# peterdavidfagan/mujoco_robot_environments

Measured on AMD Instinct MI355X. Metric: env steps/sec (whole node), RearrangementEnv batch=4096 at 1/2/4/8 MI355X, higher is better.
Workload: dtype f32

## Files before the change

include/mre.h:

```cpp
#ifndef MRE_H
#define MRE_H
#include <stddef.h>
#include <stdint.h>
#ifdef __cplusplus
extern "C" {
#endif

#define MRE_NQ 43
#define MRE_NV 39
#define MRE_NU 8
#define MRE_NQ_PAD 44
#define MRE_TRACE_W 88
#define MRE_TRACE_QVEL 48
#define MRE_NV_PAD 40
#define MRE_MAX_PROPS 4

typedef enum {
  MRE_OK = 0,
  MRE_ERR_ARG = -1,
  MRE_ERR_MODEL = -2,
  MRE_ERR_HIP = -3,
  MRE_ERR_NOGPU = -4
} mre_status;

// ... 107 lines not shown

#define MRE_SRC_RED 0
#define MRE_SRC_GREEN 1
#define MRE_SRC_BLUE 2
#define MRE_SRC_HEIGHT 3
#define MRE_F32 0
#define MRE_BF16 1
int mre_warp_inputs(void* stream, const float* hmap, const uint8_t* cmap, int n, int in_h, int in_w,
                    const int32_t* index, const float* mats, int samples, int out_h, int out_w,
                    int channels, const int32_t* chan_src, const float* chan_scale, const float* chan_bias,
                    int dtype, void* out);

int mre_correlate_workspace(int n, int rotations, int h, int w, size_t* bytes);
int mre_correlate(void* stream, const uint16_t* scene, const uint16_t* kern, int n, int rotations, int depth,
                  int h, int w, int crop, int dtype, void* logits, int64_t* best_index, float* best_value,
                  void* workspace, size_t workspace_bytes);

#define MRE_SOLVER_PGS 0
#define MRE_SOLVER_NEWTON 2
int mre_set_solver(mre_env*, int solver);
int mre_get_solver(mre_env*);
int mre_get_fallback_stats(mre_env*, long long* out4);
int mre_get_queue_info(mre_env*, long long* out5);

int mre_profile_enable(mre_env*, int on);
int mre_profile_read(mre_env*, float* total_ms, int* launches);

#ifdef __cplusplus
}
#endif
#endif
```

mujoco_robot_environments_amd/csrc/mre_api.cpp:

```cpp
#include <hip/hip_runtime.h>

#include <cmath>
#include <cstdio>
#include <cstdlib>
#include <cstring>
#include <string>
#include <algorithm>
#include <vector>

#include "mre_env.h"
#include "mre_labels.h"
#include "mre_heightmap.h"
#include "mre_warp.h"
#include "mre_warp_inputs.h"
#include "mre_correlate.h"
#include "mre_launch.h"
#include "mre_model.h"
#include "mre_records.h"

using namespace mre;

static thread_local std::string g_err;
int mre::fail(int code, const std::string& msg) {
  g_err = msg;
// ... 722 lines not shown
  if (!e) return fail(MRE_ERR_ARG, "null handle");
  DRAIN(e);
  if (solver != MRE_SOLVER_PGS && solver != MRE_SOLVER_NEWTON)
    return fail(MRE_ERR_ARG, "mre_set_solver: solver is 0 (PGS) or 2 (Newton)");
  HIPCHK(hipSetDevice(e->device));
  HIPCHK(hipStreamSynchronize(e->stream));
  e->solver = solver;
  return MRE_OK;
}

extern "C" int mre_get_solver(mre_env* e) {
  if (!e) return fail(MRE_ERR_ARG, "null handle");
  return e->solver;
}

extern "C" int mre_get_queue_info(mre_env* e, long long* out5) {
  if (!e || !out5) return fail(MRE_ERR_ARG, "mre_get_queue_info: null");
  DRAIN(e);
  out5[0] = e->n_queue_launches; out5[1] = e->queue_waves; out5[2] = e->queue_ticks; out5[3] = e->queue_ok ? 1 : 0;
  out5[4] = e->n_handovers;
  return MRE_OK;
}

extern "C" int mre_get_fallback_stats(mre_env* e, long long* out4) {
  if (!e || !out4) return fail(MRE_ERR_ARG, "mre_get_fallback_stats: null");
  DRAIN(e);
  out4[0] = e->n_large; out4[1] = e->n_reruns; out4[2] = e->n_promotions; out4[3] = e->n_demotions;
  return MRE_OK;
}

extern "C" int mre_set_state(mre_env* e, const float* qpos, const float* qvel) {
  if (!e) return fail(MRE_ERR_ARG, "null handle");
  DRAIN(e);
  int rc = MRE_OK;
  if (qpos) rc = copy_in(e, e->qpos, qpos, (size_t)e->N * NQP * 4);
  if (!rc && qvel) rc = copy_in(e, e->qvel, qvel, (size_t)e->N * NVP * 4);
  if (!rc && qpos) {
    HIPCHK(hipMemset2DAsync(e->qfine, QFINE_ROW * 4, 0, QFINE * 2, (size_t)e->N, e->stream));
    HIPCHK(hipMemset2DAsync(e->qfine + QFINE_CUBE_Q, QFINE_ROW * 4, 0, (QFINE_CUBE_V - QFINE_CUBE_Q) * 4, (size_t)e->N, e->stream));
  }
  if (!rc && qvel) {
    HIPCHK(hipMemset2DAsync(e->qfine + QFINE / 2, QFINE_ROW * 4, 0, QFINE * 2, (size_t)e->N, e->stream));
    HIPCHK(hipMemset2DAsync(e->qfine + QFINE_CUBE_V, QFINE_ROW * 4, 0, (QFINE_ROW - QFINE_CUBE_V) * 4, (size_t)e->N, e->stream));
  }
  return rc;
}
// ... 691 lines not shown
```

mujoco_robot_environments_amd/csrc/mre_dev.h:

```cpp
#pragma once
#include <stdint.h>

namespace mre {

constexpr int NB = 20;
constexpr int NRB = 16;
constexpr int GRIP_BODY0 = 8;
constexpr int NV = 39;
constexpr int NRV = 15;
constexpr int NQ = 43;
constexpr int NQP = 44;
constexpr int TRACE_W = 88;
constexpr int TRACE_QVEL = 48;
constexpr int NVP = 40;
constexpr int NU = 8;
constexpr int QFINE = 32;
constexpr int QFINE_ROW = 96;
constexpr int QFINE_CUBE_Q = 32;
constexpr int QFINE_CUBE_V = 60;
static_assert(QFINE_CUBE_Q + 7 * 4 == QFINE_CUBE_V && QFINE_CUBE_V + 6 * 4 <= QFINE_ROW, "qfine row layout");
constexpr int NPROP = 4;
constexpr int NG = 20;
constexpr int PROP_GEOM0 = 12;
constexpr int NPAIR = 128;
// ... 186 lines not shown
  float* contacts_full;
  int* settle_steps;
  int min_settle_steps;
  const uint8_t* large;
  int want_large;
  float *sv_qpos, *sv_qvel, *sv_qacc_ws, *sv_qfine, *sv_ctrl;
  int* sv_nstep;
  uint32_t* sv_status;
  uint8_t* sv_converged;
  int* launch_info;
  uint8_t* pending;
  int* q_head;
  int* q_tail;
  int* q_buf;
  int* q_acc;
  int* q_done;
  int* q_started;
  const int* q_gen;
  int q_gen_expect;
  int q_wait;
  int* q_err;
  int q_nticks, q_shards, q_cap, q_stride;
  int q_lshards, q_capl;
};
constexpr int QUEUE_TICKS_MAX = 256;
constexpr int QUEUE_SHARDS_MAX = 32;
constexpr int QUEUE_LSHARDS_MAX = 16;

struct SearchArgs {
  const DevModel* M;
  int N;
  float* qpos;
  const int* nprops;
  const float* prop_size;
  const uint8_t* env_mask;
  const long long* env_ids;
  long long env_id_offset;
  unsigned long long seed;
  const int* prop;
  int fixed_prop;
  const double* bounds;
  double shared_bounds[6];
  const int* tick_base;
  long long tick0;
  int max_attempts;
  int yaw_mode;
// ... 60 lines not shown
```

mujoco_robot_environments_amd/csrc/mre_env.h:

```cpp
#pragma once
#include <hip/hip_runtime.h>

#include <string>
#include <utility>
#include <vector>

#include "../../include/mre.h"
#include "mre_dev.h"
#include "mre_policy.h"

#define HIPCHK(x)                                                                       \
  do {                                                                                  \
    hipError_t e_ = (x);                                                                \
    if (e_ != hipSuccess)                                                               \
      return mre::fail(MRE_ERR_HIP, std::string(#x) + ": " + hipGetErrorString(e_));    \
  } while (0)

struct mre_env {
  int N = 0, device = 0;
  hipStream_t stream = nullptr;
  mre::DevModel* dM = nullptr;
  mre::DevModel hM;
  int solver = MRE_SOLVER_PGS;
  float *qpos = nullptr, *qvel = nullptr, *qacc_ws = nullptr, *ctrl = nullptr;
// ... 76 lines not shown
  bool queue_ok = true;
  int queue_ticks = 200;
  int queue_waves = 0;
  int queue_shards = 16;
  int queue_lshards = 8;
  bool queue_test_serial = false;
  int queue_spare_large = 8;
  int queue_run_ticks = 100;
  int queue_min_ticks = 32;
  float tick_tail = 0.f;
  bool tick_tail_valid = false;
  float queue_tail_min = 1.45f;
  unsigned tail_samples = 0;
  std::vector<int> tail_scratch;
  int queue_large_waves_max = 0;
  int* h_qlist = nullptr;
  int* q_ws = nullptr;
  int* q_gen = nullptr;
  int* h_q_err = nullptr;
  int* h_qgrp_order = nullptr;
  long n_queue_launches = 0;
  long long n_handovers = 0;
  int queue_last_handovers = 0;
  static constexpr int RING = mre::policy::RING;
  int ring = 2;
  static constexpr int NSTAGE = mre::policy::NSTAGE;
  hipEvent_t ev_main = nullptr;
  float* seq_copy[RING + 1] = {nullptr, nullptr, nullptr, nullptr, nullptr};
  size_t seq_cap = 0;
  unsigned seq_calls = 0;
  double dbg_wait_s = 0, dbg_call_s = 0; long dbg_calls = 0;
  int calls_since_drain = 0, sync_streak = 0;
  bool broken = false;
};

namespace mre {
int fail(int code, const std::string& msg);
int sched_create(mre_env* e);
void sched_destroy(mre_env* e);
int launch_step(mre_env* e, const StepArgs& a, bool settle = false, bool pipeline_ok = true, bool allow_queue = false);
int drain(mre_env* e, bool api_call = false);
}
#define DRAIN(e) do { int rc_ = mre::drain(e, true); if (rc_) return rc_; } while (0)
#define DRAIN_PENDING(e) do { int rc_ = mre::drain(e, false); if (rc_) return rc_; } while (0)

inline int profile_events(mre_env* e, hipEvent_t* e0, hipEvent_t* e1) {
// ... 12 lines not shown
```

mujoco_robot_environments_amd/csrc/mre_kernels.hip:

```cpp
#include <hip/hip_runtime.h>

#include "mre_dev.h"
#include "mre_math.h"
#include "mre_collide.h"

namespace mre {
using ModelP = MRE_MODEL_PTR(DevModel);
#if defined(MRE_PHASE_STAMPS) && MRE_PHASE_STAMPS >= 4
__shared__ unsigned long long dbg_acc[4];
#endif

struct OscSm {
  float J[6][7], M[7][7], MiJt[7][6], Li[6][6], Lam[6][6], V[6][6], Jbar[7][6];
  float ep[3], eo[3], F[6], LF[6], tn[7], Jbt[6], xd[6], w[6];
};

struct alignas(8) Blk {
  uint16_t row0;
  uint8_t type, nrows;
  uint8_t rslot;
  uint8_t pa, pb;
  uint8_t primary : 4;
  uint8_t bslot : 4;
};
// ... 1248 lines not shown
    }
  }
  for (int k = 0; k < S; ++k) {
    const int sh = home + k < S ? home + k : home + k - S;
    const int r = queue_pop_shard(a, l, sh, env, tick);
    if (r != 0) { shard = sh; return r > 0; }
  }
  return false;
}
MRE_DEV void queue_push(const StepArgs& a, int l, int env, int tick, int shard) {
  __builtin_amdgcn_fence(__ATOMIC_RELEASE, "agent");
  asm volatile("s_waitcnt vmcnt(0)" ::: "memory");
  if (l == 0) {
    const int i = __hip_atomic_fetch_add(a.q_tail + shard * QUEUE_TICKS_MAX + tick, 1, __ATOMIC_RELAXED, __HIP_MEMORY_SCOPE_AGENT);
    __hip_atomic_store(q_bucket(a, tick, shard) + i, env + 1, __ATOMIC_RELAXED, __HIP_MEMORY_SCOPE_AGENT);
  }
}

template <bool QUEUE>
MRE_DEV void step_body(const StepArgs& a, Sm& s) {
  OscSm& osc = s.osc;
  const int l = threadIdx.x;
  int env = 0, qtick = 0, qshard = 0;
  if (!QUEUE) {
    if ((int)blockIdx.x >= a.N) return;
    env = a.env_order != nullptr ? a.env_order[blockIdx.x] : (int)blockIdx.x;
  }
  if (QUEUE && !Q_LARGE && l == 0) __hip_atomic_fetch_add(a.q_started, 1, __ATOMIC_RELAXED, __HIP_MEMORY_SCOPE_AGENT);
  if (QUEUE && Q_LARGE && a.q_wait != 0) {
    for (unsigned idle = 0; q_load(a.q_gen) != a.q_gen_expect; ++idle) {
      if (idle > 1024u) return;
      __builtin_amdgcn_s_sleep(127);
    }
  }
 for (;;) {
  if (QUEUE) {
    if (!queue_pop(a, l, (int)(blockIdx.x % (unsigned)(Q_LARGE ? a.q_lshards : a.q_shards)), env, qtick, qshard)) return;
    if (qtick > 0 || Q_LARGE) __builtin_amdgcn_fence(__ATOMIC_ACQUIRE, "agent");
  }
  const int step_lo = QUEUE ? qtick * a.control_steps : 0, step_hi = QUEUE ? step_lo + a.control_steps : a.nsteps;
  if (QUEUE && !Q_LARGE && qtick == 0 && a.large != nullptr && a.large[env] != 0) continue;
  if (!QUEUE || (!Q_LARGE && qtick == 0)) {
#define MRE_PASS_SKIP { if (QUEUE) { if (l == 0) __hip_atomic_fetch_add(a.q_done, 1, __ATOMIC_RELAXED, __HIP_MEMORY_SCOPE_AGENT); continue; } return; }
  if (!QUEUE && a.large != nullptr && (a.large[env] != 0) != (a.want_large != 0)) return;
  if (a.env_mask != nullptr && a.env_mask[env] == 0) {
    if (a.launch_info != nullptr && l < 4) a.launch_info[(size_t)env * 4 + l] = -1;
    MRE_PASS_SKIP;
  }
  if (a.pending != nullptr && a.pending[env] != 0) {
    if (a.launch_info != nullptr && l < 4) a.launch_info[(size_t)env * 4 + l] = l == 0 ? -2 : -1;
    MRE_PASS_SKIP;
  }
#undef MRE_PASS_SKIP
  }
  ModelP M = (ModelP)a.M;

  const bool save = a.sv_qpos != nullptr && step_lo == 0;
  if (l < NQP) {
    const float v = a.qpos[(size_t)env * NQP + l];
    s.qpos[l] = v;
    if (save) a.sv_qpos[(size_t)env * NQP + l] = v;
  }
  if (l < NVP) {
    const float v = a.qvel[(size_t)env * NVP + l], w = a.qacc_ws[(size_t)env * NVP + l];
    s.qvel[l] = v;
    s.qacc[l] = w;
    s.qfrc_con[l] = 0.f;
    if (save) { a.sv_qvel[(size_t)env * NVP + l] = v; a.sv_qacc_ws[(size_t)env * NVP + l] = w; }
  }
  if (l < QFINE) {
    const float v = a.qfine != nullptr ? a.qfine[(size_t)env * QFINE_ROW + l] : 0.f;
    s.qlo[l] = v;
    if (save && a.qfine != nullptr) a.sv_qfine[(size_t)env * QFINE_ROW + l] = v;
  }
  if (save && a.qfine != nullptr && l < QFINE_ROW - QFINE)
    a.sv_qfine[(size_t)env * QFINE_ROW + QFINE + l] = a.qfine[(size_t)env * QFINE_ROW + QFINE + l];
  float cube_lo_keep = 0.f;
  if (QUEUE && !Q_LARGE && a.qfine != nullptr && l < QFINE_ROW - QFINE) cube_lo_keep = a.qfine[(size_t)env * QFINE_ROW + QFINE + l];
  if (l < NU) {
    const float v = a.ctrl[(size_t)env * NU + l];
    s.ctrl[l] = v;
    if (save) a.sv_ctrl[(size_t)env * NU + l] = v;
  }
  if (save && l == 0) {
    if (a.nstep != nullptr) a.sv_nstep[env] = a.nstep[env];
    a.sv_status[env] = a.status[env];
    a.sv_converged[env] = a.converged != nullptr ? a.converged[env] : (uint8_t)0;
  }
  if (l == 0) { s.nprops = a.nprops[env]; s.overflow = 0; s.ncon = 0; s.nefc = 0; s.solver_iters = 0; }
#ifdef MRE_NEWTON
  if (l < 24) s.zrow[l] = 0.f;
#endif
  if (l < NPROP * 3) {
    const float sz = a.prop_size[(size_t)env * NPROP * 3 + l];
    s.prop_size[l / 3][l % 3] = sz;
  }
  MRE_SYNC();
  if (l < NPROP) {
    const float m = M->body_mass[NRB + l];
    const float* z = s.prop_size[l];
    s.prop_mass[l] = m;
    s.prop_inertia[l][0] = m / 3.f * (z[1] * z[1] + z[2] * z[2]);
    s.prop_inertia[l][1] = m / 3.f * (z[0] * z[0] + z[2] * z[2]);
    s.prop_inertia[l][2] = m / 3.f * (z[0] * z[0] + z[1] * z[1]);
  }
  MRE_SYNC();

#if defined(MRE_PHASE_STAMPS) && MRE_PHASE_STAMPS >= 4
  if (l < 4) dbg_acc[l] = 0ull;
#endif
#ifdef MRE_PHASE_STAMPS
  unsigned long long stamp_acc[4] = {0, 0, 0, 0};
  unsigned long long stamp_t = __builtin_amdgcn_s_memtime();
#endif
  bool arm_converged = ((a.flags & F_CONV_CONTINUE) != 0 || (QUEUE && qtick > 0)) && a.converged != nullptr && a.converged[env] != 0;
  float grip_cmd = 0.f;
  const OscConfig* oscp = a.osc + (size_t)env * a.osc_stride;
  int hw_ncon = 0, hw_nefc = 0, hw_nrrow = 0, hw_npp = 0;
  const unsigned long long launch_t0 = __builtin_amdgcn_s_memtime();
  if (a.mode == CTRL_OSC) {
    if (l < 16) s.osc_tgt[l] = a.osc_target[(size_t)env * 16 + l];
    grip_cmd = a.grip_closed[env] ? M->act_ctrlrange[NU - 1][1] : M->act_ctrlrange[NU - 1][0];
    MRE_SYNC();
  }
  int steps_done = 0;
  bool settled = false;
  for (int step = step_lo; step < step_hi; ++step) {
    MRE_STAMP(7);
    position_stage(M, s, l);
    MRE_STAMP(12);
    MRE_STAMP(13);
    gripper_local(M, s, l);
    if ((a.flags & F_NO_CONSTRAINTS) == 0) connect_rows_local(M, s, l);
    MRE_STAMP(14);
    crb_mass_matrix(M, s, l);
    MRE_SYNC();
#ifndef MRE_NEWTON
    factor_robot_regs(s.qM, s.qLD, s.qLDinv);
#endif
    MRE_STAMP(15);
    MRE_STAMP(0);

// ... 161 lines not shown
  }
  if (a.sites != nullptr && q_last) {
    float* o = a.sites + (size_t)env * 16;
    if (l < 3) o[l] = s.site_xpos[M->opt_rec.tcp_site][l];
    if (l >= 3 && l < 6) o[l] = s.site_xpos[M->opt_rec.eef_site][l - 3];
    if (l == 6) {
      float q[4];
      mat2q(q, s.site_xmat[0]);
      o[6] = q[0]; o[7] = q[1]; o[8] = q[2]; o[9] = q[3];
    }
  }
  if (hand_over) {
    if (a.qfine != nullptr && l < QFINE_ROW - QFINE) a.qfine[(size_t)env * QFINE_ROW + QFINE + l] = cube_lo_keep;
  } else {
    if (l < NQP) a.qpos[(size_t)env * NQP + l] = s.qpos[l];
    if (l < NVP) {
      a.qvel[(size_t)env * NVP + l] = s.qvel[l];
      a.qacc_ws[(size_t)env * NVP + l] = l < NV ? s.qacc[l] : 0.f;
    }
    if (l < QFINE && a.qfine != nullptr) a.qfine[(size_t)env * QFINE_ROW + l] = s.qlo[l];
    if (l < NU) a.ctrl[(size_t)env * NU + l] = s.ctrl[l];
  }
  const bool q_more = QUEUE && !hand_over && qtick + 1 < a.q_nticks;
  if (l == 0 && a.launch_info != nullptr) {
    int* li = a.launch_info + (size_t)env * 4;
    unsigned long long dt = (__builtin_amdgcn_s_memtime() - launch_t0) >> 10;
    int moved = 0;
    if (QUEUE) {
      int* qa = a.q_acc + (size_t)env * 4;
      if (qtick > 0 || Q_LARGE) {
        hw_ncon = max(hw_ncon, q_load(qa + 0) & 0xFFFF); hw_nefc = max(hw_nefc, q_load(qa + 1));
        hw_nrrow = max(hw_nrrow, q_load(qa + 2) & 0xFFFF); hw_npp = max(hw_npp, q_load(qa + 2) >> 16);
        dt += (unsigned long long)q_load(qa + 3);
        moved = q_load(qa + 0) >> 16;
      }
      if (hand_over) moved = 1;
      if (q_more || hand_over) { qa[0] = hw_ncon | (moved << 16); qa[1] = hw_nefc; qa[2] = hw_nrrow | (hw_npp << 16); qa[3] = (int)dt; }
      else dt /= (unsigned long long)(qtick + 1);
    }
    if (!q_more && !hand_over) {
#ifdef MRE_LARGE_CAPS
      li[0] = (s.overflow ? 2 : 0) | (moved ? 4 : 0);
#else
      li[0] = s.overflow ? 1 : 0;
#endif
      li[1] = hw_ncon | ((int)(dt < 0x7FFFull ? dt : 0x7FFFull) << 16); li[2] = hw_nefc; li[3] = hw_nrrow | (hw_npp << 16);
    }
  }
#ifndef MRE_LARGE_CAPS
  if (!QUEUE && l == 0 && a.pending != nullptr && s.overflow) a.pending[env] = 1;
#endif
  if (l == 0 && a.status != nullptr && !hand_over) {
    unsigned st = 0;
    for (int k = 0; k < NQ; k++) if (!isfinite(s.qpos[k])) st |= 2u;
    if (s.overflow) st |= 4u;
    if (QUEUE) { if (st) __hip_atomic_fetch_or(a.status + env, st, __ATOMIC_RELAXED, __HIP_MEMORY_SCOPE_AGENT); }
    else a.status[env] |= st;
    if (a.stats != nullptr && a.nsteps > 0) {
      a.stats[env * 4 + 0] = s.ncon; a.stats[env * 4 + 1] = s.nefc;
      a.stats[env * 4 + 2] = s.solver_iters; a.stats[env * 4 + 3] = s.nl;
#ifdef MRE_PHASE_STAMPS
      for (int k = 0; k < 4; k++) a.stats[env * 4 + k] = (int)(stamp_acc[k] >> 4);
#if MRE_PHASE_STAMPS >= 4
      for (int k = 0; k < 4; k++) a.stats[env * 4 + k] = (int)(dbg_acc[k] >> 4);
#endif
#endif
    }
  }
  if (!QUEUE) return;
  if (hand_over) queue_push(a, l, env, qtick, a.q_shards + env % a.q_lshards);
  else if (q_more) queue_push(a, l, env, qtick + 1, qshard);
  else if (l == 0) __hip_atomic_fetch_add(a.q_done, 1, __ATOMIC_RELAXED, __HIP_MEMORY_SCOPE_AGENT);
 }
}

#ifdef MRE_NEWTON
#define MRE_VARIANT(name) name##_newton
#else
#define MRE_VARIANT(name) name
#endif

#ifdef MRE_LARGE_CAPS
__global__ __launch_bounds__(64, 2) void MRE_VARIANT(k_step_large)(StepArgs a) {
  __shared__ Sm s;
  step_body<false>(a, s);
}
}

extern "C" void MRE_VARIANT(mre_launch_step_large)(const mre::StepArgs* args, hipStream_t stream) {
  hipLaunchKernelGGL(mre::MRE_VARIANT(k_step_large), dim3(args->N), dim3(64), 0, stream, *args);
}
namespace mre {
// ... 379 lines not shown
```

mujoco_robot_environments_amd/csrc/mre_policy.h:

```cpp
#pragma once
#include <algorithm>

#include "mre_dev.h"

namespace mre {
namespace policy {

constexpr int RING = 4;
constexpr int NSTAGE = RING + 1;

inline int info_duration(const int* li) { return li[0] < 0 ? 0 : (li[1] >> 16); }

inline int compact_nrrow_max(bool newton) { return newton ? NRROW_MAX_COMPACT_NEWTON : NRROW_MAX_COMPACT_PGS; }
inline bool near_compact_caps(bool newton, int hw_ncon, int hw_nefc, int hw_nrrow, int hw_npp) {
  return 8 * hw_ncon > 7 * NCON_MAX || 8 * hw_nefc > 7 * NEFC_MAX || 8 * hw_nrrow > 7 * compact_nrrow_max(newton) || 8 * hw_npp > 7 * NPP_MAX;
}
inline bool far_below_compact_caps(bool newton, int hw_ncon, int hw_nefc, int hw_nrrow, int hw_npp) {
  return 8 * hw_ncon <= 5 * NCON_MAX && 8 * hw_nefc <= 5 * NEFC_MAX && 8 * hw_nrrow <= 5 * compact_nrrow_max(newton) && 8 * hw_npp <= 5 * NPP_MAX;
}

enum Action {
  NONE,
  RERUN,
  PROMOTE,
// ... 45 lines not shown
  return fs;
}

inline int queue_large_waves(const int* info_last, const uint8_t* large, int lo, int n, int nl, int last_handovers,
                             int spare_large, int large_waves_max ) {
  int lw = nl + std::max(last_handovers, spare_large);
  double wl = 0, wc = 0;
  for (int i = lo; i < lo + n; i++) {
    const double d = (double)info_duration(info_last + 4 * (size_t)i);
    if (large[i]) wl += d; else wc += d;
  }
  const double ncomp = (double)(n - nl);
  const double r = (wl > 0 && wc > 0) ? wl / wc : (ncomp > 0 ? 1.3 * (double)nl / ncomp : 1e9);
  const double x = r * 160.0 / (26.5 * r + 20.4);
  const int bal = std::max((int)(x * (double)(large_waves_max / 2)), large_waves_max / 4);
  return std::max(std::min(lw, bal), 1);
}

inline bool queue_fits(bool queue_ok, int queue_waves, int N) { return queue_ok && queue_waves > 0 && N > queue_waves; }
inline bool window_wants_queue(int nticks, int queue_min_ticks, bool tick_tail_valid, float tick_tail, float queue_tail_min) {
  return nticks >= queue_min_ticks || (nticks >= 8 && !(tick_tail_valid && tick_tail < queue_tail_min));
}

inline int ring_keep(int nsteps, int ring) { return nsteps <= 50 ? ring - 1 : 0; }

}
}
```

mujoco_robot_environments_amd/csrc/mre_sched.cpp:

```cpp
#include <hip/hip_runtime.h>
#include <chrono>
#include <cstdlib>
#include <cstring>

#include "mre_env.h"
#include "mre_launch.h"

using namespace mre;

static void launch_compact(const mre_env* e, const StepArgs& a, hipStream_t st, bool settle = false) {
  const StepKernels& K = step_kernels(e->solver);
  (settle ? K.settle : K.step)(&a, st);
}
static void launch_large(const mre_env* e, const StepArgs& a, hipStream_t st) { step_kernels(e->solver).large(&a, st); }

static int launch_split(const mre_env* e, const StepArgs& a, bool run_large, bool settle, hipStream_t st, hipStream_t st2,
                        hipEvent_t ev_fork, hipEvent_t ev_join) {
  StepArgs ac = a;
  ac.want_large = 0;
  if (run_large) {
    HIPCHK(hipEventRecord(ev_fork, st));
    HIPCHK(hipStreamWaitEvent(st2, ev_fork, 0));
    StepArgs al = a;
    al.want_large = 1;
// ... 30 lines not shown
}

static int process_oldest(mre_env* e, mre_env::Group& G) {
  if (G.nout == 0) return MRE_OK;
  const int slot = G.head;
  mre_env::Group::Out& O = G.out[slot];
  {
    const auto w0 = std::chrono::steady_clock::now();
    HIPCHK(hipEventSynchronize(O.ev_info));
    e->dbg_wait_s += std::chrono::duration<double>(std::chrono::steady_clock::now() - w0).count();
  }
  if (e->h_q_err && *e->h_q_err != 0) {
    e->broken = true;
    return fail(MRE_ERR_HIP, "queue launch: an env listed as ready never arrived (internal error)");
  }
  const int* const info = e->h_launch_info + (size_t)slot * 4 * (size_t)e->N;
  int younger[mre_env::RING];
  for (int k = 1; k < G.nout; k++) younger[k - 1] = G.out[(slot + k) % mre_env::RING].stage;
  const int fs = policy::free_stage(G.cur, younger, G.nout - 1);
  int* const order_stage = G.h_order + (size_t)fs * (size_t)e->N;
  bool changed = false;
  const long long handovers0 = e->n_handovers;
  const int nrerun = apply_launch_info(e, info, G.lo, G.n, &changed);
  if (&G == &e->qgroup) e->queue_last_handovers = (int)(e->n_handovers - handovers0);
  else if (O.args.nsteps == O.args.control_steps && (e->tail_samples++ & 3u) == 0u && G.n >= 256) {
    float ratio;
    e->tail_scratch.resize((size_t)G.n);
    if (policy::tick_tail_ratio(info, G.lo, G.n, e->tail_scratch.data(), &ratio)) {
      e->tick_tail = e->tick_tail_valid ? 0.9f * e->tick_tail + 0.1f * ratio : ratio;
      e->tick_tail_valid = true;
    }
  }
  if (policy::sort_longest_first(info, G.lo, G.n, order_stage) == 0)
    memcpy(order_stage + G.lo, G.h_order + (size_t)G.cur * (size_t)e->N + G.lo, (size_t)G.n * 4);
  if (nrerun > 0) {
    int rc = restore_rerun_rows(e, G.lo, G.n, e->d_pending, G.st);
    if (rc) return rc;
    for (int k = 0; k < G.nout; k++) {
      StepArgs ar = G.out[(slot + k) % mre_env::RING].args;
      ar.env_mask = e->mask_r; ar.launch_info = nullptr; ar.large = nullptr; ar.sv_qpos = nullptr; ar.pending = nullptr;
      ar.q_head = nullptr;
      launch_large(e, ar, G.st);
      HIPCHK(hipGetLastError());
    }
    e->n_reruns += nrerun;
  }
  memcpy(e->h_large_stage + (size_t)fs * (size_t)e->N + G.lo, e->h_large.data() + G.lo, (size_t)G.n);
// ... 59 lines not shown
  if (p0) HIPCHK(hipEventRecord(p0, G.st));
  guard_args(e, a);
  a.pending = e->d_pending;
  const int slot = (G.head + G.nout) % mre_env::RING;
  a.large = e->d_large_stage + (size_t)G.cur * N;
  a.launch_info = e->d_launch_info + (size_t)slot * 4 * N;
  const uint8_t* const fl = e->h_large_stage + (size_t)G.cur * N;
  if (queue) {
    StepArgs ac = a;
    ac.want_large = 0;
    const StepKernels& K = step_kernels(e->solver);
    const int nt = a.nsteps / a.control_steps, S = e->queue_shards, cap = (G.n + S - 1) / S;
    const int SL = e->queue_lshards, capl = (G.n + SL - 1) / SL;
    constexpr int QS = QUEUE_SHARDS_MAX + QUEUE_LSHARDS_MAX;
    const size_t ctl = 2 * (size_t)QS * QUEUE_TICKS_MAX + 16;
    const size_t stride = (size_t)S * cap + (size_t)SL * capl;
    const size_t words = ctl + 4 * N + (size_t)nt * stride;
    ac.sv_qpos = nullptr;
    ac.q_head = e->q_ws; ac.q_tail = ac.q_head + QS * QUEUE_TICKS_MAX;
    ac.q_done = ac.q_tail + QS * QUEUE_TICKS_MAX; ac.q_started = ac.q_done + 1; ac.q_acc = ac.q_done + 16;
    ac.q_buf = ac.q_acc + 4 * N; ac.q_err = e->h_q_err; ac.q_nticks = nt; ac.q_shards = S; ac.q_cap = cap; ac.q_stride = (int)stride;
    ac.q_lshards = SL; ac.q_capl = capl;
    ac.q_gen = e->q_gen; ac.q_gen_expect = (int)(e->n_queue_launches + 1);
    int* const hl = e->h_qlist + (size_t)(e->n_queue_launches % (mre_env::RING + 1)) * (N + 32);
    int nl = 0;
    for (int j = 0; j < SL; j++) hl[j] = 0;
    memset(hl + 16, 0, (size_t)SL * capl * 4);
    for (int i = G.lo; i < G.lo + G.n; i++)
      if (fl[i]) { const int j = i % SL; hl[16 + (size_t)j * capl + hl[j]++] = i + 1; nl++; }
    StepArgs al = ac;
    al.want_large = 1; al.q_wait = 1;
    const int lw = policy::queue_large_waves(e->h_info_last, fl, G.lo, G.n, nl, e->queue_last_handovers, e->queue_spare_large,
                                             e->queue_large_waves_max);
    hipStream_t const st_large = e->queue_test_serial ? G.st : G.st2;
    K.queue_large(&al, lw, st_large);
    HIPCHK(hipGetLastError());
    HIPCHK(hipEventRecord(G.ev_join, st_large));
    HIPCHK(hipMemsetAsync(e->q_ws, 0, ((words * 4 + 15) / 16) * 16, G.st));
    if (nl > 0) {
      HIPCHK(hipMemcpyAsync(ac.q_buf + (size_t)S * cap, hl + 16, (size_t)SL * capl * 4, hipMemcpyHostToDevice, G.st));
      HIPCHK(hipMemcpy2DAsync(ac.q_tail + S * QUEUE_TICKS_MAX, (size_t)QUEUE_TICKS_MAX * 4, hl, 4, 4, (size_t)SL, hipMemcpyHostToDevice, G.st));
    }
    HIPCHK(hipMemsetD32Async((hipDeviceptr_t)e->q_gen, ac.q_gen_expect, 1, G.st));
    const int nwaves = G.n < e->queue_waves ? G.n : e->queue_waves;
    K.queue(&ac, nwaves, G.st);
    HIPCHK(hipGetLastError());
    al.q_wait = 0;
    const int sweep = G.n < 3 * e->queue_large_waves_max ? G.n : 3 * e->queue_large_waves_max;
    K.queue_large(&al, sweep, G.st);
    e->n_queue_launches++;
    HIPCHK(hipGetLastError());
    HIPCHK(hipStreamWaitEvent(G.st, G.ev_join, 0));
  } else {
    bool run_large = false;
    for (int i = G.lo; i < G.lo + G.n && !run_large; i++) run_large = fl[i] != 0;
    rc = launch_split(e, a, run_large, false, G.st, G.st2, G.ev_fork, G.ev_join);
    if (rc) return rc;
  }
  if (p1) HIPCHK(hipEventRecord(p1, G.st));
  HIPCHK(hipEventRecord(G.out[slot].ev_info, G.st));
  G.out[slot].args = a;
  G.out[slot].stage = G.cur;
  G.nout++;
  return MRE_OK;
}
static int launch_group(mre_env* e, mre_env::Group& G, const StepArgs& a_full, bool queue = false) {
  while (G.nout > policy::ring_keep(a_full.nsteps, e->ring)) {
    int rc = process_oldest(e, G);
    if (rc) return rc;
  }
  int rc = launch_group_enqueue(e, G, a_full, queue);
  if (rc) {
    (void)hipStreamSynchronize(G.st);
    (void)hipStreamSynchronize(G.st2);
    G.nout = 0; G.head = 0;
// ... 108 lines not shown
  e->groups.resize(ng);
  auto& Q = e->qgroup;
  Q.lo = 0; Q.n = num_envs;
  HIPCHK(hipHostMalloc((void**)&e->h_qgrp_order, mre_env::NSTAGE * N * 4, hipHostMallocMapped | hipHostMallocCoherent));
  Q.h_order = e->h_qgrp_order;
  HIPCHK(hipHostGetDevicePointer((void**)&Q.d_order, Q.h_order, 0));
  for (int k = 0; k < mre_env::NSTAGE; k++)
    for (int i = 0; i < num_envs; i++) Q.h_order[(size_t)k * N + i] = i;
  HIPCHK(hipStreamCreateWithPriority(&Q.st, hipStreamNonBlocking, least));
  HIPCHK(hipStreamCreateWithPriority(&Q.st2, hipStreamNonBlocking, greatest));
  HIPCHK(hipEventCreateWithFlags(&Q.ev_fork, hipEventDisableTiming));
  HIPCHK(hipEventCreateWithFlags(&Q.ev_join, hipEventDisableTiming));
  for (auto& o : Q.out) HIPCHK(hipEventCreateWithFlags(&o.ev_info, hipEventDisableTiming));
  if (const char* q = getenv("MRE_QUEUE")) e->queue_ok = atoi(q) != 0;
  if (const char* q = getenv("MRE_QUEUE_TICKS")) { const int v = atoi(q); if (v >= 2 && v <= QUEUE_TICKS_MAX) e->queue_ticks = v; }
  if (e->queue_run_ticks > e->queue_ticks) e->queue_run_ticks = e->queue_ticks;
  hipDeviceProp_t prop;
  HIPCHK(hipGetDeviceProperties(&prop, e->device));
  e->queue_waves = prop.multiProcessorCount * std::min(step_kernels(MRE_SOLVER_PGS).queue_waves_per_cu(),
                                                       step_kernels(MRE_SOLVER_NEWTON).queue_waves_per_cu());
  if (const char* q = getenv("MRE_QUEUE_WAVES")) { const int v = atoi(q); if (v > 0) e->queue_waves = v; }
  if (const char* q = getenv("MRE_QUEUE_SHARDS")) { const int v = atoi(q); if (v >= 1 && v <= QUEUE_SHARDS_MAX) e->queue_shards = v; }
  if (const char* q = getenv("MRE_QUEUE_MIN_TICKS")) { const int v = atoi(q); if (v >= 2) e->queue_min_ticks = v; }
  if (const char* q = getenv("MRE_QUEUE_TAIL_MIN")) { const float v = (float)atof(q); if (v > 0.f) e->queue_tail_min = v; }
  if (const char* q = getenv("MRE_QUEUE_TEST_SERIAL")) e->queue_test_serial = atoi(q) != 0;
  if (const char* q = getenv("MRE_QUEUE_SPARE_LARGE")) { const int v = atoi(q); if (v >= 0) e->queue_spare_large = v; }
  e->queue_large_waves_max = 2 * prop.multiProcessorCount;
  if (const char* q = getenv("MRE_QUEUE_LSHARDS")) { const int v = atoi(q); if (v >= 1 && v <= QUEUE_LSHARDS_MAX) e->queue_lshards = v; }
  HIPCHK(hipMalloc(&e->q_ws, ((2 * (size_t)(QUEUE_SHARDS_MAX + QUEUE_LSHARDS_MAX) * QUEUE_TICKS_MAX + 16 + 4 * N +
                               (size_t)QUEUE_TICKS_MAX * (2 * N + QUEUE_SHARDS_MAX + QUEUE_LSHARDS_MAX)) * 4 + 15) / 16 * 16));
  HIPCHK(hipMalloc(&e->q_gen, 64));
  HIPCHK(hipMemsetAsync(e->q_gen, 0, 64, e->stream));
  HIPCHK(hipHostMalloc((void**)&e->h_qlist, (size_t)(mre_env::RING + 1) * (N + 32) * 4, hipHostMallocDefault));
  HIPCHK(hipHostMalloc((void**)&e->h_q_err, 64, hipHostMallocMapped | hipHostMallocCoherent));
  *e->h_q_err = 0;
  for (int g = 0; g < ng; g++) {
    auto& G = e->groups[g];
    G.h_order = e->h_grp_order; G.d_order = e->d_grp_order;
    G.lo = (int)((long long)num_envs * g / ng);
    G.n = (int)((long long)num_envs * (g + 1) / ng) - G.lo;
    int pr = 0;
    const char* gp = getenv("MRE_GROUP_PRIORITY");
    if (!(gp && atoi(gp) == 0)) { pr = greatest + g; if (pr > least) pr = least; }
    if (const char* map = getenv("MRE_GROUP_PRIO_MAP")) {
      if ((int)strlen(map) > g && map[g] >= '0' && map[g] <= '9') { pr = greatest + (map[g] - '0'); if (pr > least) pr = least; }
    }
// ... 28 lines not shown
```

mujoco_robot_environments_amd/lib.py:

```python
from __future__ import annotations

import ctypes as C
import os
import shutil
import subprocess
from typing import Optional

_CSRC = os.path.join(os.path.dirname(os.path.abspath(__file__)), "csrc")
_SO = os.path.join(_CSRC, "libmre.so")
_SOURCES = ["mre_kernels.hip", "mre_render.hip", "mre_api.cpp"]
_HEADERS = ["mre_dev.h", "mre_math.h", "mre_collide.h", "mre_solver.h", "mre_newton.h", "mre_osc.h",
            os.path.join("..", "..", "include", "mre.h")]
_UNHASHED_SOURCES = ["mre_records.hip", "mre_records.h", "mre_labels.hip", "mre_labels.h", "mre_heightmap.hip", "mre_heightmap.h",
                     "mre_heightmap_point.h", "mre_warp.hip", "mre_warp.h", "mre_warp_point.h", "mre_warp_inputs.hip", "mre_warp_inputs.h",
                     "mre_warp_input_point.h", "mre_correlate.hip", "mre_correlate.h", "mre_model.cpp", "mre_model.h", "mre_sched.cpp", "mre_env.h",
                     "mre_policy.h", "mre_launch.h"]
_LIB: Optional[C.CDLL] = None

MRE_NQ, MRE_NV, MRE_NU, MRE_NQ_PAD, MRE_NV_PAD, MRE_MAX_PROPS = 43, 39, 8, 44, 40, 4
MRE_TRACE_W = 88
MRE_TRACE_QVEL = 48
MRE_FINAL_W = 83
MRE_DYN_W = 128

EXPORTS = [
    "mre_create", "mre_destroy", "mre_last_error", "mre_num_envs", "mre_stream", "mre_sync",
    "mre_set_props", "mre_reset", "mre_place_props", "mre_set_state", "mre_get_state", "mre_get_ctrl",
    "mre_set_warmstart", "mre_get_warmstart", "mre_set_ctrl", "mre_step", "mre_rollout", "mre_rollout_ticks",
    "mre_set_trace", "mre_osc_set_target", "mre_osc_configure", "mre_gripper_set",
    "mre_run_controller", "mre_get_sites", "mre_get_status", "mre_get_solver_stats",
    "mre_profile_enable", "mre_profile_read", "mre_set_env_id_offset", "mre_set_env_order",
    "mre_set_fallback", "mre_get_fallback_stats", "mre_get_queue_info", "mre_set_solver", "mre_get_solver", "mre_wait_stream", "mre_osc_compute", "mre_get_contacts", "mre_get_contacts_full", "mre_get_settle_steps", "mre_get_launch_info", "mre_prop_place", "mre_sort_colours", "mre_crc32c", "mre_osc_configure_env", "mre_set_env_ids", "mre_set_render_colours", "mre_render",
    "mre_get_state_f64", "mre_set_state_f64", "mre_get_time", "mre_pack_final_state",
    "mre_records_workspace_bytes", "mre_varint_pack_rows", "mre_crc32c_rows", "mre_crc32c_combine",
    "mre_varint_unpack_workspace_bytes", "mre_varint_unpack_rows", "mre_get_arm_dynamics", "mre_seg_labels",
    "mre_heightmap", "mre_warp_maps", "mre_warp_inputs", "mre_correlate_workspace", "mre_correlate",
]
MRE_UNPACK_LONG, MRE_UNPACK_OVERFLOW, MRE_UNPACK_TRUNCATED, MRE_UNPACK_COUNT, MRE_UNPACK_DESC = 1, 2, 4, 8, 16


class MreError(RuntimeError):
    pass


def source_hash() -> str:
    import hashlib
    h = hashlib.sha256()
    for f in sorted(f for f in _SOURCES + _HEADERS if not f.endswith(("mre_api.cpp", "mre.h"))):
        with open(os.path.join(_CSRC, f), "rb") as fh:
            h.update(f.encode() + b"\0" + fh.read())
    return h.hexdigest()[:16]


def needs_build() -> bool:
    if not os.path.exists(_SO):
        return True
    t = os.path.getmtime(_SO)
    for f in _SOURCES + _HEADERS + _UNHASHED_SOURCES:
        p = os.path.join(_CSRC, f)
        if os.path.exists(p) and os.path.getmtime(p) > t:
# ... 74 lines not shown
    L.mre_get_solver_stats.argtypes = [vp, fp]
    L.mre_set_env_id_offset.argtypes = [vp, C.c_longlong]
    L.mre_set_env_ids.argtypes = [vp, C.POINTER(C.c_longlong)]
    L.mre_set_env_order.argtypes = [vp, fp]
    L.mre_profile_enable.argtypes = [vp, ci]
    L.mre_profile_read.argtypes = [vp, C.POINTER(C.c_float), C.POINTER(ci)]
    L.mre_set_fallback.argtypes = [vp, ci]
    L.mre_set_solver.argtypes = [vp, ci]
    L.mre_get_solver.argtypes = [vp]
    L.mre_wait_stream.argtypes = [vp, vp]
    L.mre_osc_compute.argtypes = [vp, fp, fp]
    L.mre_get_arm_dynamics.argtypes = [vp, ci, fp]
    L.mre_get_contacts.argtypes = [vp, fp, fp]
    L.mre_get_contacts_full.argtypes = [vp, ci, fp, fp]
    L.mre_get_settle_steps.argtypes = [vp, fp]
    L.mre_get_launch_info.argtypes = [vp, fp]
    L.mre_prop_place.argtypes = [vp, C.c_uint64, fp, fp, fp, ci, C.c_float, fp, fp]
    L.mre_sort_colours.argtypes = [vp, C.c_uint64, fp, fp, ci, C.c_float, fp, fp, fp, fp]
    L.mre_set_render_colours.argtypes = [vp, fp, fp]
    L.mre_render.argtypes = [vp, fp, fp, C.c_float, ci, ci, fp, fp, fp, fp]
    L.mre_osc_configure_env.argtypes = [vp, fp, fp, fp]
    L.mre_get_fallback_stats.argtypes = [vp, C.POINTER(C.c_longlong)]
    L.mre_get_queue_info.argtypes = [vp, C.POINTER(C.c_longlong)]
    sz = C.c_size_t
    L.mre_crc32c.restype = C.c_uint32
    L.mre_crc32c.argtypes = [C.c_char_p, sz]
    L.mre_crc32c_combine.restype = C.c_uint32
    L.mre_crc32c_combine.argtypes = [C.c_uint32, C.c_uint32, sz]
    L.mre_records_workspace_bytes.restype = sz
    L.mre_records_workspace_bytes.argtypes = [ci, sz]
    L.mre_varint_pack_rows.argtypes = [vp, fp, sz, sz, fp, ci, ci, fp, sz, fp, fp, fp, fp, sz]
    L.mre_crc32c_rows.argtypes = [vp, fp, sz, sz, fp, ci, ci, fp, fp, sz]
    L.mre_varint_unpack_workspace_bytes.restype = sz
    L.mre_varint_unpack_workspace_bytes.argtypes = [ci, sz]
    L.mre_varint_unpack_rows.argtypes = [vp, fp, sz, fp, fp, fp, fp, ci, sz, fp, sz, fp, fp, sz]
    L.mre_seg_labels.argtypes = [vp, fp, fp, ci, ci, ci, ci, ci, fp, fp]
    L.mre_heightmap.argtypes = [vp, fp, fp, fp, ci, ci, ci, fp, fp, C.c_float, C.c_float, ci, ci, fp, fp, fp, fp]
    L.mre_warp_maps.argtypes = [vp, fp, fp, fp, ci, ci, ci, fp, fp, ci, ci, ci, fp, fp, fp, fp]
    L.mre_warp_inputs.argtypes = [vp, fp, fp, ci, ci, ci, fp, fp, ci, ci, ci, ci, fp, fp, fp, ci, fp]
    L.mre_correlate_workspace.argtypes = [ci, ci, ci, ci, C.POINTER(sz)]
    L.mre_correlate.argtypes = [vp, fp, fp, ci, ci, ci, ci, ci, ci, ci, fp, fp, fp, fp, sz]
    for name in EXPORTS:
        if name not in ("mre_last_error", "mre_stream", "mre_crc32c", "mre_crc32c_combine",
                        "mre_records_workspace_bytes", "mre_varint_unpack_workspace_bytes"):
            getattr(L, name).restype = ci
    _LIB = L
    return L


def check(rc: int, what: str = "") -> None:
    if rc != 0:
        msg = lib().mre_last_error()
        raise MreError(f"{what} failed ({rc}): {msg.decode() if msg else ''}")
```

mujoco_robot_environments_amd/physics.py:

```python
from __future__ import annotations

import ctypes as C
from typing import Optional, Sequence, Tuple

import numpy as np
import torch

from . import lib as _lib
from .lib import MRE_NQ, MRE_NQ_PAD, MRE_NU, MRE_NV, MRE_NV_PAD, MRE_MAX_PROPS, MRE_TRACE_W, check
from .model import compile as _compile

FLAG_NO_CONSTRAINTS = 1
FLAG_FREEZE_ROBOT = 2


def _ptr(t) -> Optional[int]:
    if t is None:
        return None
    if isinstance(t, torch.Tensor):
        assert t.is_contiguous()
        return t.data_ptr()
    if isinstance(t, np.ndarray):
        assert t.flags["C_CONTIGUOUS"]
        return t.ctypes.data
# ... 347 lines not shown
        n = self.num_envs
        t_rgb = torch.empty((n, height, width, 3), dtype=torch.uint8, device=self.device) if rgb else None
        t_depth = torch.empty((n, height, width), dtype=torch.float32, device=self.device) if depth else None
        t_seg = torch.empty((n, height, width), dtype=torch.uint8, device=self.device) if seg else None
        cp = np.ascontiguousarray(cam_pos, np.float32).reshape(3)
        cm = np.ascontiguousarray(cam_mat, np.float32).reshape(9)
        m = None if mask is None else np.ascontiguousarray(mask, np.uint8)
        check(_lib.lib().mre_render(self._h, _ptr(cp), _ptr(cm), float(fovy), int(height), int(width),
                                    _ptr(t_rgb), _ptr(t_depth), _ptr(t_seg), _ptr(m)), "mre_render")
        self.sync()
        return t_rgb, t_depth, t_seg

    def set_fallback(self, mode=True) -> None:
        check(_lib.lib().mre_set_fallback(self._h, int(mode)), "mre_set_fallback")

    def fallback_stats(self) -> dict:
        out = (C.c_longlong * 4)()
        check(_lib.lib().mre_get_fallback_stats(self._h, out), "mre_get_fallback_stats")
        return {"large_envs": int(out[0]), "reruns": int(out[1]), "promotions": int(out[2]), "demotions": int(out[3])}

    def queue_info(self) -> dict:
        out = (C.c_longlong * 5)()
        check(_lib.lib().mre_get_queue_info(self._h, out), "mre_get_queue_info")
        return {"launches": int(out[0]), "waves": int(out[1]), "ticks_per_launch": int(out[2]), "enabled": bool(out[3]),
                "handovers": int(out[4])}

    def profile_enable(self, on: bool = True) -> None:
        check(_lib.lib().mre_profile_enable(self._h, int(on)), "mre_profile_enable")

    def profile_read(self):
        ms, n = C.c_float(0), C.c_int(0)
        check(_lib.lib().mre_profile_read(self._h, C.byref(ms), C.byref(n)), "mre_profile_read")
        return float(ms.value), int(n.value)
```

Before: 25.83 million.

## Keep env state resident in LDS across consecutive queue ticks

In the persistent queue kernel, a block that finishes a tick can now continue straight into the next tick for the same env, up to a hold count (default 2). It skips the queue push/pop, the global-memory reload of qpos/qvel/ctrl/prop data and the launch-info write. The goal is less atomic queue traffic and less memory round-tripping per tick. In exchange, load balancing across blocks gets coarser, the hold is disabled near the end of the launch to limit tail imbalance, and a device-to-host copy of a counter is added.

```diff
diff --git a/include/mre.h b/include/mre.h
--- a/include/mre.h
+++ b/include/mre.h
@@ -153,6 +153,7 @@
 int mre_get_solver(mre_env*);
 int mre_get_fallback_stats(mre_env*, long long* out4);
 int mre_get_queue_info(mre_env*, long long* out5);
+int mre_get_queue_hold_info(mre_env*, long long* out2);
 
 int mre_profile_enable(mre_env*, int on);
 int mre_profile_read(mre_env*, float* total_ms, int* launches);
diff --git a/mujoco_robot_environments_amd/csrc/mre_api.cpp b/mujoco_robot_environments_amd/csrc/mre_api.cpp
--- a/mujoco_robot_environments_amd/csrc/mre_api.cpp
+++ b/mujoco_robot_environments_amd/csrc/mre_api.cpp
@@ -768,6 +768,13 @@
   return MRE_OK;
 }
 
+extern "C" int mre_get_queue_hold_info(mre_env* e, long long* out2) {
+  if (!e || !out2) return fail(MRE_ERR_ARG, "mre_get_queue_hold_info: null");
+  DRAIN(e);
+  out2[0] = e->n_held_ticks; out2[1] = e->queue_hold;
+  return MRE_OK;
+}
+
 extern "C" int mre_get_fallback_stats(mre_env* e, long long* out4) {
   if (!e || !out4) return fail(MRE_ERR_ARG, "mre_get_fallback_stats: null");
   DRAIN(e);
diff --git a/mujoco_robot_environments_amd/csrc/mre_dev.h b/mujoco_robot_environments_amd/csrc/mre_dev.h
--- a/mujoco_robot_environments_amd/csrc/mre_dev.h
+++ b/mujoco_robot_environments_amd/csrc/mre_dev.h
@@ -232,6 +232,8 @@
   int* q_err;
   int q_nticks, q_shards, q_cap, q_stride;
   int q_lshards, q_capl;
+  int q_hold, q_hold_until;
+  int* q_held;
 };
 constexpr int QUEUE_TICKS_MAX = 256;
 constexpr int QUEUE_SHARDS_MAX = 32;
diff --git a/mujoco_robot_environments_amd/csrc/mre_env.h b/mujoco_robot_environments_amd/csrc/mre_env.h
--- a/mujoco_robot_environments_amd/csrc/mre_env.h
+++ b/mujoco_robot_environments_amd/csrc/mre_env.h
@@ -122,6 +122,8 @@
   long n_queue_launches = 0;
   long long n_handovers = 0;
   int queue_last_handovers = 0;
+  int queue_hold = 0;
+  long long n_held_ticks = 0;
   static constexpr int RING = mre::policy::RING;
   int ring = 2;
   static constexpr int NSTAGE = mre::policy::NSTAGE;
diff --git a/mujoco_robot_environments_amd/csrc/mre_kernels.hip b/mujoco_robot_environments_amd/csrc/mre_kernels.hip
--- a/mujoco_robot_environments_amd/csrc/mre_kernels.hip
+++ b/mujoco_robot_environments_amd/csrc/mre_kernels.hip
@@ -1294,6 +1294,9 @@
   OscSm& osc = s.osc;
   const int l = threadIdx.x;
   int env = 0, qtick = 0, qshard = 0;
+  int q_run = 0, q_nheld = 0;
+  int hw_ncon = 0, hw_nefc = 0, hw_nrrow = 0, hw_npp = 0;
+  unsigned long long launch_t0 = 0ull;
   if (!QUEUE) {
     if ((int)blockIdx.x >= a.N) return;
     env = a.env_order != nullptr ? a.env_order[blockIdx.x] : (int)blockIdx.x;
@@ -1306,8 +1309,12 @@
     }
   }
  for (;;) {
-  if (QUEUE) {
-    if (!queue_pop(a, l, (int)(blockIdx.x % (unsigned)(Q_LARGE ? a.q_lshards : a.q_shards)), env, qtick, qshard)) return;
+  const bool held = QUEUE && q_run > 0;
+  if (QUEUE && !held) {
+    if (!queue_pop(a, l, (int)(blockIdx.x % (unsigned)(Q_LARGE ? a.q_lshards : a.q_shards)), env, qtick, qshard)) {
+      if (l == 0 && q_nheld > 0) __hip_atomic_fetch_add(a.q_held, q_nheld, __ATOMIC_RELAXED, __HIP_MEMORY_SCOPE_AGENT);
+      return;
+    }
     if (qtick > 0 || Q_LARGE) __builtin_amdgcn_fence(__ATOMIC_ACQUIRE, "agent");
   }
   const int step_lo = QUEUE ? qtick * a.control_steps : 0, step_hi = QUEUE ? step_lo + a.control_steps : a.nsteps;
@@ -1328,6 +1335,13 @@
   ModelP M = (ModelP)a.M;
 
   const bool save = a.sv_qpos != nullptr && step_lo == 0;
+  if (held) {
+    if (l < NVP) {
+      if (l >= NV) s.qacc[l] = 0.f;
+      s.qfrc_con[l] = 0.f;
+    }
+    if (l < QFINE && a.qfine == nullptr) s.qlo[l] = 0.f;
+  } else {
   if (l < NQP) {
     const float v = a.qpos[(size_t)env * NQP + l];
     s.qpos[l] = v;
@@ -1347,9 +1361,10 @@
   }
   if (save && a.qfine != nullptr && l < QFINE_ROW - QFINE)
     a.sv_qfine[(size_t)env * QFINE_ROW + QFINE + l] = a.qfine[(size_t)env * QFINE_ROW + QFINE + l];
+  }
   float cube_lo_keep = 0.f;
   if (QUEUE && !Q_LARGE && a.qfine != nullptr && l < QFINE_ROW - QFINE) cube_lo_keep = a.qfine[(size_t)env * QFINE_ROW + QFINE + l];
-  if (l < NU) {
+  if (!held && l < NU) {
     const float v = a.ctrl[(size_t)env * NU + l];
     s.ctrl[l] = v;
     if (save) a.sv_ctrl[(size_t)env * NU + l] = v;
@@ -1359,16 +1374,16 @@
     a.sv_status[env] = a.status[env];
     a.sv_converged[env] = a.converged != nullptr ? a.converged[env] : (uint8_t)0;
   }
-  if (l == 0) { s.nprops = a.nprops[env]; s.overflow = 0; s.ncon = 0; s.nefc = 0; s.solver_iters = 0; }
+  if (l == 0) { if (!held) s.nprops = a.nprops[env]; s.overflow = 0; s.ncon = 0; s.nefc = 0; s.solver_iters = 0; }
 #ifdef MRE_NEWTON
   if (l < 24) s.zrow[l] = 0.f;
 #endif
-  if (l < NPROP * 3) {
+  if (!held && l < NPROP * 3) {
     const float sz = a.prop_size[(size_t)env * NPROP * 3 + l];
     s.prop_size[l / 3][l % 3] = sz;
   }
   MRE_SYNC();
-  if (l < NPROP) {
+  if (!held && l < NPROP) {
     const float m = M->body_mass[NRB + l];
     const float* z = s.prop_size[l];
     s.prop_mass[l] = m;
@@ -1388,8 +1403,7 @@
   bool arm_converged = ((a.flags & F_CONV_CONTINUE) != 0 || (QUEUE && qtick > 0)) && a.converged != nullptr && a.converged[env] != 0;
   float grip_cmd = 0.f;
   const OscConfig* oscp = a.osc + (size_t)env * a.osc_stride;
-  int hw_ncon = 0, hw_nefc = 0, hw_nrrow = 0, hw_npp = 0;
-  const unsigned long long launch_t0 = __builtin_amdgcn_s_memtime();
+  if (!held) { hw_ncon = 0; hw_nefc = 0; hw_nrrow = 0; hw_npp = 0; launch_t0 = __builtin_amdgcn_s_memtime(); }
   if (a.mode == CTRL_OSC) {
     if (l < 16) s.osc_tgt[l] = a.osc_target[(size_t)env * 16 + l];
     grip_cmd = a.grip_closed[env] ? M->act_ctrlrange[NU - 1][1] : M->act_ctrlrange[NU - 1][0];
@@ -1597,7 +1611,8 @@
     if (l < NU) a.ctrl[(size_t)env * NU + l] = s.ctrl[l];
   }
   const bool q_more = QUEUE && !hand_over && qtick + 1 < a.q_nticks;
-  if (l == 0 && a.launch_info != nullptr) {
+  const bool q_keep = QUEUE && q_more && q_run + 1 < a.q_hold && qtick + 1 < a.q_hold_until;
+  if (l == 0 && a.launch_info != nullptr && !q_keep) {
     int* li = a.launch_info + (size_t)env * 4;
     unsigned long long dt = (__builtin_amdgcn_s_memtime() - launch_t0) >> 10;
     int moved = 0;
@@ -1643,6 +1658,13 @@
     }
   }
   if (!QUEUE) return;
+  if (q_keep) {
+    q_run++; q_nheld++; qtick++;
+    hw_ncon = __builtin_amdgcn_readfirstlane(hw_ncon); hw_nefc = __builtin_amdgcn_readfirstlane(hw_nefc);
+    hw_nrrow = __builtin_amdgcn_readfirstlane(hw_nrrow); hw_npp = __builtin_amdgcn_readfirstlane(hw_npp);
+    continue;
+  }
+  q_run = 0;
   if (hand_over) queue_push(a, l, env, qtick, a.q_shards + env % a.q_lshards);
   else if (q_more) queue_push(a, l, env, qtick + 1, qshard);
   else if (l == 0) __hip_atomic_fetch_add(a.q_done, 1, __ATOMIC_RELAXED, __HIP_MEMORY_SCOPE_AGENT);
diff --git a/mujoco_robot_environments_amd/csrc/mre_policy.h b/mujoco_robot_environments_amd/csrc/mre_policy.h
--- a/mujoco_robot_environments_amd/csrc/mre_policy.h
+++ b/mujoco_robot_environments_amd/csrc/mre_policy.h
@@ -91,6 +91,16 @@
   return nticks >= queue_min_ticks || (nticks >= 8 && !(tick_tail_valid && tick_tail < queue_tail_min));
 }
 
+constexpr int QUEUE_HOLD_DEFAULT = 2;
+inline int queue_hold_ticks(int n_ticks, int knob) {
+  if (n_ticks < 2) return 1;
+  return std::min(knob > 0 ? knob : QUEUE_HOLD_DEFAULT, n_ticks);
+}
+inline int queue_hold_until(int n_ticks, int hold) {
+  if (hold <= 1) return 0;
+  return n_ticks - std::min(hold, std::max(1, n_ticks / 4));
+}
+
 inline int ring_keep(int nsteps, int ring) { return nsteps <= 50 ? ring - 1 : 0; }
 
 }
diff --git a/mujoco_robot_environments_amd/csrc/mre_sched.cpp b/mujoco_robot_environments_amd/csrc/mre_sched.cpp
--- a/mujoco_robot_environments_amd/csrc/mre_sched.cpp
+++ b/mujoco_robot_environments_amd/csrc/mre_sched.cpp
@@ -76,7 +76,10 @@
   bool changed = false;
   const long long handovers0 = e->n_handovers;
   const int nrerun = apply_launch_info(e, info, G.lo, G.n, &changed);
-  if (&G == &e->qgroup) e->queue_last_handovers = (int)(e->n_handovers - handovers0);
+  if (&G == &e->qgroup) {
+    e->queue_last_handovers = (int)(e->n_handovers - handovers0);
+    if (O.args.q_hold > 1) e->n_held_ticks += e->h_q_err[8 + slot];
+  }
   else if (O.args.nsteps == O.args.control_steps && (e->tail_samples++ & 3u) == 0u && G.n >= 256) {
     float ratio;
     e->tail_scratch.resize((size_t)G.n);
@@ -182,6 +185,10 @@
     ac.q_buf = ac.q_acc + 4 * N; ac.q_err = e->h_q_err; ac.q_nticks = nt; ac.q_shards = S; ac.q_cap = cap; ac.q_stride = (int)stride;
     ac.q_lshards = SL; ac.q_capl = capl;
     ac.q_gen = e->q_gen; ac.q_gen_expect = (int)(e->n_queue_launches + 1);
+    ac.q_held = ac.q_done + 2;
+    ac.q_hold = policy::queue_hold_ticks(nt, e->queue_hold);
+    ac.q_hold_until = policy::queue_hold_until(nt, ac.q_hold);
+    a.q_hold = ac.q_hold;
     int* const hl = e->h_qlist + (size_t)(e->n_queue_launches % (mre_env::RING + 1)) * (N + 32);
     int nl = 0;
     for (int j = 0; j < SL; j++) hl[j] = 0;
@@ -211,6 +218,7 @@
     e->n_queue_launches++;
     HIPCHK(hipGetLastError());
     HIPCHK(hipStreamWaitEvent(G.st, G.ev_join, 0));
+    if (ac.q_hold > 1) HIPCHK(hipMemcpyAsync(e->h_q_err + 8 + slot, ac.q_held, 4, hipMemcpyDeviceToHost, G.st));
   } else {
     bool run_large = false;
     for (int i = G.lo; i < G.lo + G.n && !run_large; i++) run_large = fl[i] != 0;
@@ -365,6 +373,7 @@
   if (const char* q = getenv("MRE_QUEUE_WAVES")) { const int v = atoi(q); if (v > 0) e->queue_waves = v; }
   if (const char* q = getenv("MRE_QUEUE_SHARDS")) { const int v = atoi(q); if (v >= 1 && v <= QUEUE_SHARDS_MAX) e->queue_shards = v; }
   if (const char* q = getenv("MRE_QUEUE_MIN_TICKS")) { const int v = atoi(q); if (v >= 2) e->queue_min_ticks = v; }
+  if (const char* q = getenv("MRE_QUEUE_HOLD")) { const int v = atoi(q); if (v >= 1 && v <= QUEUE_TICKS_MAX) e->queue_hold = v; }
   if (const char* q = getenv("MRE_QUEUE_TAIL_MIN")) { const float v = (float)atof(q); if (v > 0.f) e->queue_tail_min = v; }
   if (const char* q = getenv("MRE_QUEUE_TEST_SERIAL")) e->queue_test_serial = atoi(q) != 0;
   if (const char* q = getenv("MRE_QUEUE_SPARE_LARGE")) { const int v = atoi(q); if (v >= 0) e->queue_spare_large = v; }
diff --git a/mujoco_robot_environments_amd/lib.py b/mujoco_robot_environments_amd/lib.py
--- a/mujoco_robot_environments_amd/lib.py
+++ b/mujoco_robot_environments_amd/lib.py
@@ -30,12 +30,13 @@
     "mre_set_trace", "mre_osc_set_target", "mre_osc_configure", "mre_gripper_set",
     "mre_run_controller", "mre_get_sites", "mre_get_status", "mre_get_solver_stats",
     "mre_profile_enable", "mre_profile_read", "mre_set_env_id_offset", "mre_set_env_order",
-    "mre_set_fallback", "mre_get_fallback_stats", "mre_get_queue_info", "mre_set_solver", "mre_get_solver", "mre_wait_stream", "mre_osc_compute", "mre_get_contacts", "mre_get_contacts_full", "mre_get_settle_steps", "mre_get_launch_info", "mre_prop_place", "mre_sort_colours", "mre_crc32c", "mre_osc_configure_env", "mre_set_env_ids", "mre_set_render_colours", "mre_render",
+    "mre_set_fallback", "mre_get_fallback_stats", "mre_get_queue_info", "mre_get_queue_hold_info", "mre_set_solver", "mre_get_solver", "mre_wait_stream", "mre_osc_compute", "mre_get_contacts", "mre_get_contacts_full", "mre_get_settle_steps", "mre_get_launch_info", "mre_prop_place", "mre_sort_colours", "mre_crc32c", "mre_osc_configure_env", "mre_set_env_ids", "mre_set_render_colours", "mre_render",
     "mre_get_state_f64", "mre_set_state_f64", "mre_get_time", "mre_pack_final_state",
     "mre_records_workspace_bytes", "mre_varint_pack_rows", "mre_crc32c_rows", "mre_crc32c_combine",
     "mre_varint_unpack_workspace_bytes", "mre_varint_unpack_rows", "mre_get_arm_dynamics", "mre_seg_labels",
     "mre_heightmap", "mre_warp_maps", "mre_warp_inputs", "mre_correlate_workspace", "mre_correlate",
 ]
+OPTIONAL_EXPORTS = ("mre_get_queue_hold_info",)
 MRE_UNPACK_LONG, MRE_UNPACK_OVERFLOW, MRE_UNPACK_TRUNCATED, MRE_UNPACK_COUNT, MRE_UNPACK_DESC = 1, 2, 4, 8, 16
 
 
@@ -156,6 +157,8 @@
     L.mre_osc_configure_env.argtypes = [vp, fp, fp, fp]
     L.mre_get_fallback_stats.argtypes = [vp, C.POINTER(C.c_longlong)]
     L.mre_get_queue_info.argtypes = [vp, C.POINTER(C.c_longlong)]
+    if hasattr(L, "mre_get_queue_hold_info"):
+        L.mre_get_queue_hold_info.argtypes = [vp, C.POINTER(C.c_longlong)]
     sz = C.c_size_t
     L.mre_crc32c.restype = C.c_uint32
     L.mre_crc32c.argtypes = [C.c_char_p, sz]
@@ -175,6 +178,8 @@
     L.mre_correlate_workspace.argtypes = [ci, ci, ci, ci, C.POINTER(sz)]
     L.mre_correlate.argtypes = [vp, fp, fp, ci, ci, ci, ci, ci, ci, ci, fp, fp, fp, fp, sz]
     for name in EXPORTS:
+        if name in OPTIONAL_EXPORTS and not hasattr(L, name):
+            continue
         if name not in ("mre_last_error", "mre_stream", "mre_crc32c", "mre_crc32c_combine",
                         "mre_records_workspace_bytes", "mre_varint_unpack_workspace_bytes"):
             getattr(L, name).restype = ci
diff --git a/mujoco_robot_environments_amd/physics.py b/mujoco_robot_environments_amd/physics.py
--- a/mujoco_robot_environments_amd/physics.py
+++ b/mujoco_robot_environments_amd/physics.py
@@ -393,8 +393,11 @@
     def queue_info(self) -> dict:
         out = (C.c_longlong * 5)()
         check(_lib.lib().mre_get_queue_info(self._h, out), "mre_get_queue_info")
+        held = (C.c_longlong * 2)()
+        if hasattr(_lib.lib(), "mre_get_queue_hold_info"):
+            check(_lib.lib().mre_get_queue_hold_info(self._h, held), "mre_get_queue_hold_info")
         return {"launches": int(out[0]), "waves": int(out[1]), "ticks_per_launch": int(out[2]), "enabled": bool(out[3]),
-                "handovers": int(out[4])}
+                "handovers": int(out[4]), "held_ticks": int(held[0])}
 
     def profile_enable(self, on: bool = True) -> None:
         check(_lib.lib().mre_profile_enable(self._h, int(on)), "mre_profile_enable")
```

Result: faster. 26.25 million, median of 6 (+1.6%).
